# KennyRotella/delta_graph_slam

Hardware: AMD Instinct MI355X
Metric: scan registrations/sec (64k-pt pairs) (higher is better)
Workload: dtype f32 per-point, f64 accumulate; 1 GPU; cfg2 KITTI HDL-64E-shaped pairs (65,536 pts after voxel filter), NDT res 1.0 m DIRECT7, eps 0.01, max 64 iterations; 32 candidate pairs per GPU per step against one target (LoopDetector::matching, cfg4 shard), 32 distinct source scans, fitness score per candidate; inputs resident on the device before timing -- the 35 MB working set of a step fits the 256 MB Infinity Cache, so re-reads between eval; pairs_per_gpu=32, distinct_scans=32, parallelism=candidates sharded one process per GPU, all_gather of result records, collective_world_size=1

## Files before the change

### delta_graph_slam_amd/_lib.py

```python
from __future__ import annotations

import ctypes as C
import os

_HERE = os.path.dirname(os.path.abspath(__file__))
LIB_PATH = os.environ.get("DGS_REG_LIB") or os.path.join(_HERE, "libdgs_reg.so")

DGS_OK = 0
STATUS = {0: "DGS_OK", 1: "DGS_ERR_INVALID_ARGUMENT", 2: "DGS_ERR_HIP", 3: "DGS_ERR_NO_TARGET", 4: "DGS_ERR_NO_SOURCE",
          5: "DGS_ERR_GRID_TOO_LARGE", 6: "DGS_ERR_UNSUPPORTED", 7: "DGS_ERR_CAPACITY"}
DGS_ERR_CAPACITY = 7
METHOD_NDT, METHOD_GICP, METHOD_VGICP, METHOD_ICP, METHOD_PCL_GICP, METHOD_PCL_NDT = 0, 1, 2, 3, 4, 5
VGICP_SEARCH = {"DIRECT1": 0, "DIRECT7": 1, "DIRECT27": 2}
NDT_SEARCH = {"KDTREE": 0, "DIRECT26": 1, "DIRECT7": 2, "DIRECT1": 3}
NDT_ORDER = {"FAST": 0, "UPSTREAM": 1, "UPSTREAM_SEQUENTIAL": 2}
GICP_REG = {"NONE": 0, "MIN_EIG": 1, "NORMALIZED_MIN_EIG": 2, "PLANE": 3, "FROBENIUS": 4}
GICP_COV = {"SYM_EIG": 0, "JACOBI_SVD": 1, "UPSTREAM_ORDER": 2}
K_NDT_DERIVATIVES, K_NDT_SOLVE, K_NDT_VOXEL_BUILD, K_NN_SEARCH, K_GICP_LINEARIZE, K_GICP_COVARIANCE, K_TRANSFORM = range(7)


class DgsError(RuntimeError):
    def __init__(self, status: int, msg: str = ""):
        self.status = status
        super().__init__(f"{STATUS.get(status, status)}: {msg}")
# ... 145 lines not shown
PF_DOWNSAMPLE = {"NONE": 0, "VOXELGRID": 1, "APPROX_VOXELGRID": 2}
PF_OUTLIER = {"NONE": 0, "STATISTICAL": 1, "RADIUS": 2}
PF_NORM_ORDER = {"PAIRS_XY_ZW": 0, "PAIRS_XZ_YW": 1, "SEQUENTIAL": 2}


class Result(C.Structure):
    _fields_ = [("final_transformation", C.c_float * 16), ("converged", C.c_int32), ("iterations", C.c_int32),
                ("evaluations", C.c_int32), ("status", C.c_int32), ("score", C.c_double), ("fitness", C.c_double)]


SYMBOLS = [
    "dgs_params_init", "dgs_create", "dgs_destroy", "dgs_last_error", "dgs_abi_version", "dgs_set_stream",
    "dgs_synchronize", "dgs_set_input_target", "dgs_set_input_source", "dgs_align", "dgs_get_fitness_score",
    "dgs_get_inlier_fraction", "dgs_nearest_search_target", "dgs_nn_fitness_distances", "dgs_align_batch", "dgs_find_loop_candidates", "dgs_calc_fitness_score", "dgs_voxel_grid_filter", "dgs_approx_voxel_grid_filter", "dgs_cloud_create", "dgs_cloud_destroy", "dgs_cloud_size",
    "dgs_set_input_target_cloud", "dgs_set_input_source_cloud", "dgs_align_batch_clouds", "dgs_align_pairs_clouds", "dgs_profile_enable",
    "dgs_profile_get", "dgs_profile_reset", "dgs_get_counts", "dgs_ndt_derivatives", "dgs_ndt_hessian_double", "dgs_ndt_score_gradient", "dgs_deal_probe", "dgs_deal_probe_cost", "dgs_pcl_ndt_neighbours", "dgs_ndt_get_voxels",
    "dgs_ndt_get_trajectory", "dgs_gicp_get_covariances", "dgs_gicp_linearize", "dgs_vgicp_get_voxels",
    "dgs_group_create", "dgs_group_destroy", "dgs_group_last_error", "dgs_group_size", "dgs_group_uses_rccl", "dgs_group_rccl_ranks", "dgs_group_last_gather_used_rccl",
    "dgs_group_member", "dgs_group_set_input_target", "dgs_group_align_batch",
    "dgs_group_cloud_create", "dgs_group_cloud_destroy", "dgs_group_cloud_size", "dgs_group_cloud_copies", "dgs_group_cloud_trim", "dgs_group_set_input_target_cloud",
    "dgs_group_align_batch_clouds",
    "dgs_icp_options_init", "dgs_set_icp_options", "dgs_group_set_icp_options", "dgs_icp_get_trajectory",
    "dgs_pcl_gicp_options_init", "dgs_set_pcl_gicp_options", "dgs_group_set_pcl_gicp_options", "dgs_pcl_gicp_get_trajectory",
    "dgs_pcl_gicp_set_probe", "dgs_pcl_gicp_evaluate", "dgs_pcl_gicp_set_correspondence_randomness",
    "dgs_set_batch_independent", "dgs_get_batch_independent", "dgs_group_set_batch_independent",
    "dgs_prefilter_params_init", "dgs_prefilter", "dgs_prefilter_distance", "dgs_prefilter_radius", "dgs_prefilter_statistical",
    "dgs_prefilter_normal", "dgs_prefilter_get_statistics", "dgs_prefilter_get_normals",
    "dgs_prefilter_scan_params_init", "dgs_prefilter_scan", "dgs_prefilter_deskew",
    "dgs_map_cloud_params_init", "dgs_map_cloud_generate", "dgs_map_cloud_generate_clouds", "dgs_map_cloud_get", "dgs_map_cloud_get_grid",
    "dgs_line_extraction_params_init", "dgs_line_extraction", "dgs_line_extraction_get_rounds",
    "dgs_line_align_params_init", "dgs_line_align_global", "dgs_line_merge", "dgs_line_edges", "dgs_line_align_get_hypotheses",
# ... 63 lines not shown
    lib.dgs_cloud_size.argtypes = [C.c_void_p]
    lib.dgs_cloud_size.restype = C.c_int64
    lib.dgs_set_input_target_cloud.argtypes = [C.c_void_p, C.c_void_p]
    lib.dgs_set_input_source_cloud.argtypes = [C.c_void_p, C.c_void_p]
    lib.dgs_align_batch_clouds.argtypes = [C.c_void_p, C.c_int32, C.c_void_p, C.c_void_p, C.c_int32, C.c_double, P(Result)]
    lib.dgs_align_pairs_clouds.argtypes = [C.c_void_p, C.c_int32, C.c_void_p, C.c_void_p, C.c_void_p, C.c_int32, C.c_double, P(Result)]
    lib.dgs_profile_enable.argtypes = [C.c_void_p, C.c_int32]
    lib.dgs_profile_get.argtypes = [C.c_void_p, C.c_int32, P(C.c_double), P(C.c_int64)]
    lib.dgs_profile_reset.argtypes = [C.c_void_p]
    lib.dgs_get_counts.argtypes = [C.c_void_p, P(C.c_int64)]
    lib.dgs_ndt_derivatives.argtypes = [C.c_void_p, C.c_void_p, C.c_void_p, P(C.c_double), C.c_void_p, C.c_void_p]
    lib.dgs_ndt_hessian_double.argtypes = [C.c_void_p, C.c_void_p, C.c_void_p]
    lib.dgs_ndt_score_gradient.argtypes = [C.c_void_p, C.c_void_p, P(C.c_double), C.c_void_p]
    lib.dgs_deal_probe.argtypes = [C.c_void_p, C.c_void_p, C.c_int32, C.c_int32, C.c_int32, C.c_void_p]
    lib.dgs_deal_probe_cost.argtypes = [C.c_void_p, C.c_void_p, C.c_void_p, C.c_int32, C.c_int32, C.c_int32, C.c_void_p, C.c_void_p]
    lib.dgs_pcl_ndt_neighbours.argtypes = [C.c_void_p, C.c_void_p, C.c_int64, C.c_int32, C.c_void_p, C.c_void_p]
    lib.dgs_ndt_get_voxels.argtypes = [C.c_void_p, P(C.c_int64), C.c_void_p, C.c_void_p, C.c_void_p, C.c_void_p, C.c_void_p]
    lib.dgs_ndt_get_trajectory.argtypes = [C.c_void_p, C.c_int32, C.c_void_p, P(C.c_int32)]
    lib.dgs_gicp_get_covariances.argtypes = [C.c_void_p, C.c_int32, C.c_void_p]
    lib.dgs_gicp_linearize.argtypes = [C.c_void_p, C.c_void_p, C.c_int32, P(C.c_double), C.c_void_p, C.c_void_p]
    lib.dgs_vgicp_get_voxels.argtypes = [C.c_void_p, C.c_int64, C.c_void_p, C.c_void_p, C.c_void_p, C.c_void_p, P(C.c_int64)]
    lib.dgs_group_create.argtypes = [P(Params), C.c_void_p, C.c_int32, P(C.c_void_p)]
    lib.dgs_group_destroy.argtypes = [C.c_void_p]
    lib.dgs_group_destroy.restype = None
    lib.dgs_group_last_error.argtypes = [C.c_void_p]
    lib.dgs_group_last_error.restype = C.c_char_p
    lib.dgs_group_size.argtypes = [C.c_void_p]
    lib.dgs_group_uses_rccl.argtypes = [C.c_void_p]
    lib.dgs_group_rccl_ranks.argtypes = [C.c_void_p]
    lib.dgs_group_last_gather_used_rccl.argtypes = [C.c_void_p]
# ... 108 lines not shown
```

### delta_graph_slam_amd/csrc/dgs_api.hip

```cpp
#include <algorithm>
#include <cfloat>
#include <cmath>
#include <cstddef>
#include <cstdlib>
#include <cstring>
#include <new>
#include <string>
#include <vector>

#include "handle.h"

using namespace dgs;

namespace dgs {

int ensure_pinned(dgs_handle* h, size_t bytes) {
  if (bytes <= h->pinned_bytes) return DGS_OK;
  if (h->pinned) (void)hipHostFree(h->pinned);
  h->pinned = nullptr;
  h->pinned_bytes = 0;
  const size_t want = std::max<size_t>(bytes * 2, 1 << 16);
  hipError_t e = hipHostMalloc(&h->pinned, want, hipHostMallocDefault);
  if (e != hipSuccess) {
    h->err = std::string("hipHostMalloc: ") + hipGetErrorString(e);
// ... 1144 lines not shown
  if (e == hipSuccess) {
    hipLaunchKernelGGL(deal_probe_cost_kernel, dim3(grid), dim3(kBlock), 0, h->stream, d_in.ptr, d_in.ptr + n_pairs, n_pairs, cap_blocks, d_out.ptr);
    e = hipGetLastError();
  }
  if (e == hipSuccess) e = hipMemcpyAsync(out, d_out.ptr, sizeof(int4) * n_out, hipMemcpyDeviceToHost, h->stream);
  if (e == hipSuccess) e = hipStreamSynchronize(h->stream);
  d_in.release();
  d_out.release();
  if (e != hipSuccess) {
    h->err = std::string("dgs_deal_probe_cost: ") + hipGetErrorString(e);
    return DGS_ERR_HIP;
  }
  return DGS_OK;
}

int dgs_find_loop_candidates(dgs_handle* h, const double* accum_distance, const double* xy, int64_t n, int32_t on_device, double new_accum_distance,
                             const double* new_xy, double accum_distance_thresh, double distance_thresh, int32_t* indices, int64_t capacity, int64_t* n_out) {
  if (!h || !n_out || !new_xy || n < 0 || capacity < 0 || (n > 0 && (!accum_distance || !xy)) || (capacity > 0 && !indices) || n > INT32_MAX) return DGS_ERR_INVALID_ARGUMENT;
  h->err.clear();
  if (set_device(h)) return DGS_ERR_HIP;
  *n_out = 0;
  if (n == 0) return DGS_OK;
  dgs::DevBuf<double>& din = h->fc_in;
  dgs::DevBuf<int>& dout = h->fc_out;
  dgs::DevBuf<long long>& dcnt = h->fc_cnt;
  const double* d_acc = accum_distance;
  const double* d_xy = xy;
  int* d_idx = indices;
  const int64_t cap = on_device ? capacity : std::min<int64_t>(capacity, n);
  if (dcnt.reserve(1) != hipSuccess) { h->err = "hipMalloc failed"; return DGS_ERR_HIP; }
// ... 287 lines not shown
```

### delta_graph_slam_amd/csrc/handle.h

```cpp
#pragma once
#include "building_cloud.h"
#include "common.h"
#include "cov_batch_plan.h"
#include "sac.h"

namespace dgs {

struct EventPair {
  hipEvent_t start, stop;
};

struct Profiler {
  bool enabled = false;
  std::vector<EventPair> pool;
  std::vector<int> pending[DGS_K_COUNT];
  std::vector<int> weight;
  size_t next_free = 0;
  double total_ms[DGS_K_COUNT] = {0};
  int64_t launches[DGS_K_COUNT] = {0};
};

struct IcpPair;
struct IcpItem;
struct PgPair;
// ... 519 lines not shown
int stage_host_inputs(dgs_handle* h, DevBuf<float4>& slab, int n, const float* const* inputs, const int64_t* sizes, const float4** d_in);
int ensure_poll_events(dgs_handle* h);
int side_fork(dgs_handle* h);
int side_join(dgs_handle* h);
int side_build_now(dgs_handle* h);

int ndt_build_target(dgs_handle* h);
int voxel_grid_filter(dgs_handle* h, const float4* in, int64_t n, float leaf, float4* out, int64_t out_capacity, int64_t* n_out);
int approx_voxel_grid_filter(dgs_handle* h, const float4* in, int64_t n, float leaf, float4* out, int64_t out_capacity, int64_t* n_out);
int cloud_minmax(dgs_handle* h, const float4* pts, int64_t n, float out6[6]);
int cloud_minmax_device(dgs_handle* h, const float4* pts, int64_t n, float** d_out6, hipStream_t st = nullptr);
int ndt_align_pairs(dgs_handle* h, int n_pairs, const float4* const* d_src_ptrs_host, const int* sizes_host,
                    const float* guesses16, dgs_result* results);
int ndt_trajectory(dgs_handle* h, int pair, double* out, int* len);
int ndt_probe(dgs_handle* h, const double* p6, const float* T16, double* score, double* g6, double* H36, int kind = 1);
inline bool is_pcl_ndt(const dgs_handle* h) { return h->prm.method == DGS_METHOD_PCL_NDT; }
inline bool is_ndt_family(const dgs_handle* h) { return h->prm.method == DGS_METHOD_NDT || h->prm.method == DGS_METHOD_PCL_NDT; }
void pcl_ndt_launch(dgs_handle* h, int n_pairs, int cap_blocks, int total_blocks, int launch, hipStream_t st);
void pcl_ndt_init_tables(dgs_handle* h, int n_pairs, hipStream_t st);
int pcl_ndt_neighbours(dgs_handle* h, const float* queries_xyz16, int64_t m, int on_device, int32_t* counts, int32_t* voxel_ids);
int bvh_build(dgs_handle* h, Bvh& bvh, const float4* pts, int64_t n, hipStream_t st = nullptr, bool kd_order = false);
int nn_fitness(dgs_handle* h, const float4* src, int64_t n, const float* T16, double max_range, double inlier_sq,
               double* sum, int64_t* count, int64_t* inliers);
int nn_fitness_batch(dgs_handle* h, int n_pairs, const float4* const* d_src_ptrs, const int* d_sizes, int max_size, const float* d_T,
                     size_t T_stride_bytes, double max_range, double inlier_sq, double* sums, int64_t* counts, int64_t* inliers);
int nn_fitness_batch_on(dgs_handle* h, const Bvh& index, NnGrid* grid, int n_pairs, const float4* const* d_src_ptrs, const int* d_sizes, int max_size,
                        const float* d_T, size_t T_stride_bytes, double max_range, double inlier_sq, double* sums, int64_t* counts, int64_t* inliers);
int nn_fitness_prepare(dgs_handle* h, int n_pairs, int max_size, bool grid);
void nn_fitness_enqueue(dgs_handle* h, hipStream_t st, const Bvh& index, const int* ids, int count, const float4* const* d_src_ptrs, const int* d_sizes,
                        const float* d_T, size_t T_stride_bytes, double max_range, double inlier_sq, int background_lds_kb);
// ... 108 lines not shown
```

### delta_graph_slam_amd/csrc/ndt_align.hip

```cpp
#include <cfloat>
#include <cmath>
#include <cstdlib>
#include <cstring>

#include "handle.h"
#include "ndt_plan.h"
#include "solve6.h"

namespace dgs {

#include "ndt_fast.h"

#pragma clang fp contract(off)

#include "ndt_exp_tables.h"
#include "ndt_optimiser.h"
#include "ndt_strict.h"
#include "ndt_sequential.h"

__host__ __device__ inline int ndt_queue_slices(int round, int base, int cap) {
  const int f = round < 12 ? 1 : (round < 24 ? 2 : 4);
  return min(base * f, cap);
}
constexpr int kQueueHdrWords = 82;
// ... 739 lines not shown
  if (rc != DGS_OK) return rc;
  const NdtPlan P = plan_align(h);
  launch_derivatives(h, P, L, -1, kind == 2);
  launch_solve(h, P, L);
  char* base = reinterpret_cast<char*>(h->pinned);
  NdtPair* hp = reinterpret_cast<NdtPair*>(base + ((h->pinned_bytes - sizeof(NdtPair) - 64) & ~(size_t)63));
  DGS_HIP_TRY(h, hipMemcpyAsync(hp, h->pairs.ptr, sizeof(NdtPair), hipMemcpyDeviceToHost, st));
  DGS_HIP_TRY(h, hipStreamSynchronize(st));
  DGS_HIP_TRY(h, hipGetLastError());
  *score = hp->s.score;
  for (int k = 0; k < 6; k++) g6[k] = hp->s.grad[k];
  for (int k = 0; k < 36; k++) H36[k] = hp->s.hess[k];
  return DGS_OK;
}

}
```

### delta_graph_slam_amd/csrc/ndt_optimiser.h

```cpp

#ifdef DGS_NDT_PCL_DOUBLE
constexpr bool kNdtDoubleTablesAlways = true;
#else
constexpr bool kNdtDoubleTablesAlways = false;
#endif
template <bool WAVE>
__device__ __forceinline__ void trig6(const double* ang, double* sn, double* cs) {
  if (WAVE) {
    const int lane = threadIdx.x & 63;
    const double a0 = ang[0], a1 = ang[1], a2 = ang[2], a3 = ang[3], a4 = ang[4], a5 = ang[5];
    const double a = (lane == 5) ? a5 : (lane == 4) ? a4 : (lane == 3) ? a3 : (lane == 2) ? a2 : (lane == 1) ? a1 : a0;
    double sv, cv;
    sincos(a, &sv, &cv);
#pragma unroll
    for (int k = 0; k < 6; k++) { sn[k] = readlane_f64(sv, k); cs[k] = readlane_f64(cv, k); }
  } else {
#pragma unroll
    for (int k = 0; k < 6; k++) sincos(ang[k], &sn[k], &cs[k]);
  }
}

template <bool COH>
__device__ __forceinline__ void hdr_put(float* p, float v) {
  if (COH) __hip_atomic_store(p, v, __ATOMIC_RELAXED, __HIP_MEMORY_SCOPE_AGENT);
// ... 457 lines not shown
  if (strict_from_rows) {
    if (pair_blocks[pair] == 0) return;
  }
  __shared__ NdtSolver s_lds;
  NdtSolver& s = s_lds;
  __shared__ double tot[kStrictPad];
  int need_h = 0;
  if (threadIdx.x < kWave) {
    s_lds = st->s;
    need_h = st->need_hessian;
  }
  if (threadIdx.x < kStrictPad) {
    if (strict_from_rows) {
      const int nb = pair_blocks[pair];
      const double* base = partials + (size_t)pair * cap_blocks * kStrictPad + threadIdx.x;
      double v = 0.0;
      for (int b0 = 0; b0 < nb; b0 += 4) {
        double r[4];
#pragma unroll
        for (int k = 0; k < 4; k++) r[k] = base[(size_t)min(b0 + k, nb - 1) * kStrictPad];
#pragma unroll
        for (int k = 0; k < 4; k++)
          if (b0 + k < nb) v += r[k];
      }
      tot[threadIdx.x] = v;
    } else {
      tot[threadIdx.x] = strict_totals[(size_t)pair * kStrictPad + threadIdx.x];
    }
  }
  __syncthreads();
  if (threadIdx.x >= kWave) return;
  const bool writer = threadIdx.x == 0;
  if (need_h != 2) {
    s.score = tot[0];
#pragma unroll
    for (int k = 0; k < 6; k++) s.grad[k] = tot[1 + k];
  }
  if (need_h) {
#pragma unroll
    for (int k = 0; k < 36; k++) s.hess[k] = tot[7 + k];
// ... 13 lines not shown
```

### delta_graph_slam_amd/csrc/ndt_strict.h

```cpp

__device__ __forceinline__ double glibc_exp_dev(double x, const unsigned long long* __restrict__ tab) {
#pragma clang fp contract(off)
  constexpr double N = 128.0;
  constexpr double kInvLn2N = 0x1.71547652b82fep0 * N, kNegLn2hiN = -0x1.62e42fefa0000p-8, kNegLn2loN = -0x1.cf79abc9e3b3ap-47, kShift = 0x1.8p52;
  constexpr double C2 = 0x1.ffffffffffdbdp-2, C3 = 0x1.555555555543cp-3, C4 = 0x1.55555cf172b91p-5, C5 = 0x1.1111167a4d017p-7;
  const unsigned long long xb = (unsigned long long)__double_as_longlong(x);
  const unsigned abstop = (unsigned)(xb >> 52) & 0x7ffu;
  bool special = false;
  if (abstop - 0x3c9u >= 0x408u - 0x3c9u) {
    if (abstop - 0x3c9u >= 0x80000000u) return 1.0 + x;
    if (abstop >= 0x409u) {
      if (xb == 0xfff0000000000000ull) return 0.0;
      if (abstop >= 0x7ffu) return 1.0 + x;
      return (xb >> 63) ? 0.0 : __builtin_inf();
    }
    special = true;
  }
  double kd = __builtin_fma(kInvLn2N, x, kShift);
  const unsigned long long ki = (unsigned long long)__double_as_longlong(kd);
  kd -= kShift;
  const double r = __builtin_fma(kd, kNegLn2loN, __builtin_fma(kd, kNegLn2hiN, x));
  const unsigned idx = 2u * (unsigned)(ki & 127ull);
  const double tail = __longlong_as_double((long long)tab[idx]);
  unsigned long long sbits = tab[idx + 1] + (ki << 45);
// ... 368 lines not shown
  double xj[8], xh[15];
  strict_point_tables_hd(xf, StrictHeader<false>{nullptr, &st}, xj, xh);
  unsigned mask = ROWS ? ((NB >= 32) ? 0xFFFFFFFFu : ((1u << NB) - 1u)) : mask_in;
  while (mask) {
    const int k = __ffs(mask) - 1;
    mask &= mask - 1u;
    bool ok = ((mask_in >> k) & 1u) != 0;
    if (ok) ok = strict_item_hd<ROWS>(xt, xj, xh, vtab + (size_t)strict_pick(vids, k) * 12, gauss_d1, gauss_d2, acc, ROWS ? rows + k : nullptr, row_stride, exptab_d);
    if (ROWS && !ok) {
      for (int en = 0; en < 36; en++) rows[(size_t)en * row_stride + k] = 0.0;
    }
  }
}

constexpr int kStrictRowScratch = 11 * 65;
template <bool COHERENT, bool OWN_SCRATCH = true>
__device__ __forceinline__ void strict_block_row(const double (&acc)[kStrictAccum], const int ncol, double* __restrict__ row_of_slice, double* wave_scratch = nullptr) {
  constexpr int CH = 11, RS = 65, NCH = 4;
  __shared__ double tr[OWN_SCRATCH ? kBlock / kWave : 1][OWN_SCRATCH ? CH * RS : 1];
  __shared__ double sm[kBlock / kWave][kStrictPad];
  const int lane = threadIdx.x & 63, wave = threadIdx.x >> 6;
  double* my = OWN_SCRATCH ? tr[wave] : wave_scratch;
#pragma unroll
  for (int h = 0; h < NCH; h++) {
    if (h * CH >= ncol) break;
#pragma unroll
    for (int k = 0; k < CH; k++) my[k * RS + lane] = (h * CH + k < kStrictAccum) ? acc[h * CH + k < kStrictAccum ? h * CH + k : 0] : 0.0;
    __builtin_amdgcn_wave_barrier();
    __builtin_amdgcn_s_waitcnt(0xc07f);
    if (lane < CH) {
      double v = 0.0;
#pragma unroll 8
      for (int j = 0; j < 64; j++) v += my[lane * RS + j];
// ... 1 lines not shown
    }
    __builtin_amdgcn_wave_barrier();
    __builtin_amdgcn_s_waitcnt(0xc07f);
  }
  __syncthreads();
  if (threadIdx.x < kStrictPad) {
    double v = 0.0;
    if ((int)threadIdx.x < ncol) v = ((sm[0][threadIdx.x] + sm[1][threadIdx.x]) + sm[2][threadIdx.x]) + sm[3][threadIdx.x];
    double* row = row_of_slice + threadIdx.x;
    if (COHERENT) handoff_store_row(row, v);
    else *row = v;
  }
}

constexpr int kStrictSlots = 4;
__device__ __forceinline__ void strict_wave_cols(const double (&acc)[kStrictAccum], const int ncol, double* __restrict__ my, double* __restrict__ cols_of_wave) {
  constexpr int CH = 11, RS = 65, NCH = 4;
  const int lane = threadIdx.x & 63;
#pragma unroll
  for (int h = 0; h < NCH; h++) {
    if (h * CH >= ncol) break;
#pragma unroll
    for (int k = 0; k < CH; k++) my[k * RS + lane] = (h * CH + k < kStrictAccum) ? acc[h * CH + k < kStrictAccum ? h * CH + k : 0] : 0.0;
    __builtin_amdgcn_wave_barrier();
    __builtin_amdgcn_s_waitcnt(0xc07f);
    if (lane < CH) {
      double v = 0.0;
#pragma unroll 8
      for (int j = 0; j < 64; j++) v += my[lane * RS + j];
      cols_of_wave[h * CH + lane] = v;
    }
    __builtin_amdgcn_wave_barrier();
// ... 307 lines not shown
      double xj[8], xh[15];
      strict_table_read_hd<kStrictHdFields, PTS>(td, tdx, (int)(entry >> 25), xt, xj, xh);
      (void)strict_item_hd<false>(xt, xj, xh, row, gauss_d1, gauss_d2, acc, nullptr, 0, exptab_d);
    }
  }
}

constexpr int kStrictSpeculate = 1;
constexpr int kStrictDealByCost = 2;
constexpr int kStrictStampShift = 8;
#ifndef DGS_STRICT_DEAL_BY_COST
#define DGS_STRICT_DEAL_BY_COST 1
#endif

#ifdef DGS_DEAL_STAMPS
constexpr int kStampLaunches = 256, kStampGrid = 2048, kStampWords = 8;
static __device__ unsigned long long* g_deal_stamps;
#define STRICT_DEAL_STAMP_BEGIN                                                                                                        \
  const unsigned long long stamp_t0 = wall_clock64();                                                                                  \
  unsigned long long* const stamp_rec = ((flags >> kStrictStampShift) > 0 && threadIdx.x == 0 && blockIdx.x < kStampGrid && g_deal_stamps) \
      ? g_deal_stamps + ((size_t)((flags >> kStrictStampShift) - 1) * kStampGrid + blockIdx.x) * kStampWords : nullptr;
#define STRICT_DEAL_STAMP_WORK(pair, slice, kind, n_active)                                                                            \
  if (stamp_rec) {                                                                                                                     \
    stamp_rec[0] = stamp_t0;                                                                                                           \
    stamp_rec[1] = wall_clock64();                                                                                                     \
    stamp_rec[3] = (unsigned long long)blockIdx.x | ((unsigned long long)(unsigned)(pair) << 32);                                      \
    stamp_rec[4] = (unsigned long long)(unsigned)((slice) + 1) | ((unsigned long long)(unsigned)(kind) << 32);                         \
    stamp_rec[5] = (unsigned long long)(unsigned)(n_active) | ((unsigned long long)gridDim.x << 32);                                   \
  }
#define STRICT_DEAL_STAMP_CLOSED if (stamp_rec) stamp_rec[2] = wall_clock64();
#else
#define STRICT_DEAL_STAMP_BEGIN
#define STRICT_DEAL_STAMP_WORK(pair, slice, kind, n_active)
#define STRICT_DEAL_STAMP_CLOSED
#endif

template <int SEARCH, bool WITH_HD, bool RING>
struct StrictTile {
  static constexpr int NB = Offsets<SEARCH>::N;
  static constexpr int PTS = (NB <= 7) ? (WITH_HD ? 128 : 64) : 64;
  static constexpr int PTS_HD = 64;
  static constexpr int kRingOffset = kStrictFields * PTS * 4;
  static constexpr int kFloatBytes = kRingOffset + (RING ? kStrictRingBytes : 0);
  static constexpr int kQueue = PTS * NB;
  static constexpr int kHdQueueBytes = PTS_HD * NB * 4;
  static constexpr bool kHdRing = RING && WITH_HD && DGS_STRICT_HD_ITEMS != 0 && kStrictHdFields * 8 * PTS_HD + 5 * 1024 <= kFloatBytes &&
                                  kHdQueueBytes % 16 == 0 && kHdQueueBytes + 1024 + 3 * 4 * PTS_HD <= kQueue * 4;
  static constexpr int kHdFields = kHdRing ? kStrictHdFields : 23;
  static constexpr int kHdBytes = kHdRing ? kStrictHdFields * 8 * PTS_HD + 5 * 1024 : (23 * 8 + 3 * 4) * PTS_HD;
// ... 80 lines not shown
  static_assert(!TL::kHdRing || TL::kTableBytes == TL::kFloatBytes, "the double pass's ring lives in what the float kinds reserve: no more LDS than without it");
  static_assert(SEARCH != 2 || !WITH_HD || FIXED || sizeof(s_tab) + sizeof(s_queue) == 4 * (14336 + 3584), "the timed instantiation: 78,208 B of LDS per workgroup in all");
  __shared__ unsigned long long s_exp2f[32];
  constexpr bool kLdsHeader = DGS_STRICT_LDS_HEADER != 0 && !FIXED;
  __shared__ __attribute__((aligned(16))) StrictHeaderBlock s_hdr;
  {
    unsigned long long e2 = 0ull;
    if (threadIdx.x < 32) e2 = kGlibcExp2fTab[threadIdx.x];
    strict_header_word_t hw = 0u;
    const bool mine = kLdsHeader && !solver && strict_header_load(st, WITH_HD && kind == 2, hw);
    if (threadIdx.x < 32) s_exp2f[threadIdx.x] = e2;
    if (kLdsHeader) strict_header_store(&s_hdr, mine, hw);
  }
  const StrictHeader<kLdsHeader> hdr_wg{(strict_header_lds_t)&s_hdr, &st};
  __syncthreads();
  const unsigned long long* __restrict__ exptab = s_exp2f;
  const unsigned long long* __restrict__ exptab_d = kGlibcExpTab;
  const int lane = threadIdx.x & 63, wave = __builtin_amdgcn_readfirstlane((int)(threadIdx.x >> 6));
  float* tf = reinterpret_cast<float*>(s_tab[wave]);
  float4* ring = reinterpret_cast<float4*>(s_tab[wave] + TL::kRingOffset);
  unsigned* queue = s_queue[wave];
  double* td = reinterpret_cast<double*>(s_tab[wave]);
  float4* ring_hd = reinterpret_cast<float4*>(s_tab[wave] + TL::kHdFields * 8 * TL::PTS_HD);
  float4* ring_hd5 = reinterpret_cast<float4*>(reinterpret_cast<unsigned char*>(queue) + TL::kHdQueueBytes);
  float* tdx = TL::kHdRing ? reinterpret_cast<float*>(reinterpret_cast<unsigned char*>(queue) + TL::kHdQueueBytes + 1024)
                           : reinterpret_cast<float*>(s_tab[wave] + 23 * 8 * TL::PTS_HD);
  const int pts = (WITH_HD && kind == 2) ? TL::PTS_HD : TL::PTS;
  if (solver && wave == 0) {
    __shared__ NdtSolver s_x;
    NdtPair* scratch = reinterpret_cast<NdtPair*>(s_tab[0]);
// ... 5 lines not shown
    __builtin_amdgcn_s_waitcnt(0xc07f);
    __builtin_amdgcn_wave_barrier();
    bool same = queued;
    const int* pub = reinterpret_cast<const int*>(&st);
    const int* mine = reinterpret_cast<const int*>(scratch);
    for (int w = lane; w < 82; w += kWave) same = same && (pub[w] == mine[w]);
    same = __all(same) != 0;
    for (int w = lane; w < kWords; w += kWave)
      __hip_atomic_store(reinterpret_cast<double*>(&pairs[pair].spec_s) + w, reinterpret_cast<const double*>(&s_x)[w], __ATOMIC_RELAXED, __HIP_MEMORY_SCOPE_AGENT);
    if (lane == 0) __hip_atomic_store(&pairs[pair].spec_result, same ? 1 : 2, __ATOMIC_RELAXED, __HIP_MEMORY_SCOPE_AGENT);
    __builtin_amdgcn_wave_barrier();
  }
  const int subs = __builtin_amdgcn_readfirstlane(pts / 64);
  const int stride = __builtin_amdgcn_readfirstlane(n_slices * kBlock);
  static_assert(TL::kTableBytes >= kStrictRowScratch * 8, "the wave's table region doubles as its reduction scratch");
  __shared__ double s_cols[FIXED ? kStrictSlots : 1][FIXED ? kBlock / kWave : 1][FIXED ? kStrictPad : 1];
  static_assert(kStrictSlots * kStrictPad <= kBlock, "one thread per entry of the rows written together");
  int slot = 0, q_first = slice;
#pragma unroll 1
  for (int q = solver ? n_slices : slice; FIXED ? (q < n_slices) : (q == slice && !solver); q += blocks_per_pair) {
#pragma unroll
  for (int k = 0; k < kStrictAccum; k++) acc[k] = 0.0;
#pragma unroll 1
  for (int first = q * kBlock + wave * 64; first < n; first += subs * stride) {
    int qn = 0;
#pragma unroll 1
    for (int sub = 0; sub < subs; sub++) {
      const int i = first + sub * stride + lane;
      const int slot = sub * 64 + lane;
      const StrictHeader<kLdsHeader> hdr = hdr_wg.per_use();
      unsigned mask = 0;
      int vids[NB];
      if (i < n) {
        const float4 x = src[i];
        float xt[3];
        xt[0] = affine_row_rn(T[0], T[1], T[2], T[3], x.x, x.y, x.z);
        xt[1] = affine_row_rn(T[4], T[5], T[6], T[7], x.x, x.y, x.z);
        xt[2] = affine_row_rn(T[8], T[9], T[10], T[11], x.x, x.y, x.z);
        mask = strict_neighbourhood<SEARCH>(xt, g, leaf_pow2, vids);
        if (mask) {
// ... 19 lines not shown
              for (int f = 6; f < 15; f++) tf[(5 + f) * TL::PTS + slot] = xh[f];
            }
          }
        }
      }
#pragma unroll
      for (int k = 0; k < NB; k++) {
        const bool has = (mask >> k) & 1u;
        const unsigned long long b = __ballot(has);
        if (has) queue[qn + __builtin_amdgcn_mbcnt_hi((unsigned)(b >> 32), __builtin_amdgcn_mbcnt_lo((unsigned)b, 0u))] = ((unsigned)slot << 25) | (unsigned)vids[k];
        qn += __popcll(b);
      }
    }
    __builtin_amdgcn_s_waitcnt(0xc07f);
    __builtin_amdgcn_wave_barrier();
    if (!(WITH_HD && kind == 2)) {
      if (kind == 1) strict_items_float<true, TL::PTS, !FIXED>(tf, ring, queue, qn, lane, vs, gauss_d1, gd2, acc, exptab);
      else strict_items_float<false, TL::PTS, !FIXED>(tf, ring, queue, qn, lane, vs, gauss_d1, gd2, acc, exptab);
      qn = 0;
    }
    if (TL::kHdRing && kind == 2) {
      strict_items_hd<TL::PTS_HD>(td, tdx, ring_hd, ring_hd5, queue, qn, lane, vtab, gauss_d1, gauss_d2, acc, exptab_d);
      qn = 0;
    }
#pragma unroll 1
    for (int h = 0; h < qn; h += 64) {
      const int idx = h + lane;
      if (idx < qn) {
        const unsigned entry = queue[idx];
        const int slot = (int)(entry >> 25), vid = (int)(entry & 0x1FFFFFFu);
// ... 3 lines not shown
          strict_table_read_hd<23, TL::PTS_HD>(td, tdx, slot, xt, xj, xh);
          (void)strict_item_hd<false>(xt, xj, xh, vtab + (size_t)vid * 12, gauss_d1, gauss_d2, acc, nullptr, 0, exptab_d);
        } else {
          float xt[3], xj[8], xh[15];
          if (kind == 1) {
            strict_table_read<true, TL::PTS>(tf, slot, xt, xj, xh);
            strict_item<true, true>(xt, xj, xh, vs + vid, gauss_d1, gd2, acc, exptab);
          } else {
            strict_table_read<false, TL::PTS>(tf, slot, xt, xj, xh);
            strict_item<false, true>(xt, xj, xh, vs + vid, gauss_d1, gd2, acc, exptab);
          }
        }
      }
    }
    __builtin_amdgcn_wave_barrier();
  }
  if (FIXED) {
    strict_wave_cols(acc, kind ? kStrictAccum : 7, td, s_cols[slot][wave]);
    slot++;
    if (slot == kStrictSlots || q + blocks_per_pair >= n_slices) {
      strict_rows_flush<FUSED>(reinterpret_cast<const double (*)[kBlock / kWave][kStrictPad]>(&s_cols[0][0][0]), slot, kind ? kStrictAccum : 7,
                               partials + (size_t)pair * cap_blocks * kStrictPad, q_first, blocks_per_pair);
      slot = 0;
      q_first = q + blocks_per_pair;
    }
  } else {
    strict_block_row<FUSED, false>(acc, kind ? kStrictAccum : 7, partials + ((size_t)pair * cap_blocks + slice) * kStrictPad, td);
  }
  }
  if (!FUSED) return;
  __shared__ int s_last;
  if (threadIdx.x < kStrictPad) handoff_drain_stores();
  __syncthreads();
  STRICT_DEAL_STAMP_WORK(pair, slice, kind, n_active)
  const int n_tickets = blocks_per_pair + ((speculate && st.spec_pending) ? 1 : 0);
  if (threadIdx.x == 0) s_last = handoff_take_ticket(&pairs[pair].ticket, n_tickets) ? 1 : 0;
  __syncthreads();
  if (!s_last) return;
#ifdef DGS_CLOSE_STAMPS
  if (threadIdx.x == 0 && pairs[pair].s.nr_iterations == 1) pairs[pair].traj[kTrajCap - 1][5] = (double)wall_clock64();
#endif
  ndt_close_strict<false, WITH_HD>(pairs + pair, partials + (size_t)pair * cap_blocks * kStrictPad, n_slices, consts, done_flags + pair, launch, 1,
                                   solve_min_active > 0 && n_active >= solve_min_active, speculate != 0);
  STRICT_DEAL_STAMP_CLOSED
}

#ifndef DGS_NDT_PCL_DOUBLE
__global__ __launch_bounds__(kWave) void ndt_strict_solve_kernel(NdtPair* __restrict__ pairs, const int n_pairs, const NdtConsts c, int* __restrict__ done_flags, const int launch,
                                                               const int lag) {
  const int pair = blockIdx.x;
  if (pair >= n_pairs) return;
  NdtPair* st = pairs + pair;
// ... 26 lines not shown
```

### include/dgs_reg.h

```cpp
#ifndef DGS_REG_H
#define DGS_REG_H

#include <stdint.h>

#ifdef __cplusplus
extern "C" {
#endif

#define DGS_ABI_VERSION 5

typedef struct dgs_handle dgs_handle;
typedef struct dgs_cloud dgs_cloud;

enum dgs_status {
  DGS_OK = 0,
  DGS_ERR_INVALID_ARGUMENT = 1,
  DGS_ERR_HIP = 2,
  DGS_ERR_NO_TARGET = 3,
  DGS_ERR_NO_SOURCE = 4,
  DGS_ERR_GRID_TOO_LARGE = 5,
  DGS_ERR_UNSUPPORTED = 6,
  DGS_ERR_CAPACITY = 7
};

// ... 186 lines not shown

enum dgs_kernel_id {
  DGS_K_NDT_DERIVATIVES = 0, DGS_K_NDT_SOLVE = 1, DGS_K_NDT_VOXEL_BUILD = 2, DGS_K_NN_SEARCH = 3,
  DGS_K_GICP_LINEARIZE = 4, DGS_K_GICP_COVARIANCE = 5, DGS_K_TRANSFORM = 6, DGS_K_COUNT = 7
};
int dgs_profile_enable(dgs_handle* h, int32_t enable);
int dgs_profile_get(dgs_handle* h, int32_t kernel_id, double* total_ms, int64_t* launches);
int dgs_profile_reset(dgs_handle* h);
int dgs_get_counts(dgs_handle* h, int64_t out[8]);

int dgs_ndt_derivatives(dgs_handle* h, const double* p6, const float* T16, double* score, double* grad6, double* hess36);
int dgs_ndt_hessian_double(dgs_handle* h, const double* p6, double* hess36);
int dgs_ndt_score_gradient(dgs_handle* h, const double* p6, double* score, double* grad6);
int dgs_deal_probe(dgs_handle* h, const int32_t* active, int32_t n_pairs, int32_t cap_blocks, int32_t grid, int32_t* out);
int dgs_deal_probe_cost(dgs_handle* h, const int32_t* active, const int32_t* kinds, int32_t n_pairs, int32_t cap_blocks, int32_t grid, int32_t* out, int32_t* order3);
int dgs_pcl_ndt_neighbours(dgs_handle* h, const float* queries_xyz16, int64_t m, int32_t on_device, int32_t* counts, int32_t* voxel_ids);
int dgs_ndt_get_trajectory(dgs_handle* h, int32_t pair, double* poses6, int32_t* len);
int dgs_icp_get_trajectory(dgs_handle* h, int32_t pair, float* T16s, double* mse, int32_t* n_corr, int32_t capacity, int32_t* len);
int dgs_pcl_gicp_set_probe(dgs_handle* h, const float* T16, const float* guess16);
int dgs_pcl_gicp_evaluate(dgs_handle* h, const double* x6, int32_t* m, double* f, double* g6);
int dgs_pcl_gicp_get_trajectory(dgs_handle* h, int32_t pair, float* T16s, int32_t* n_corr, int32_t* inner, int32_t* passes, double* f,
                                int32_t capacity, int32_t* len);
int dgs_ndt_get_voxels(dgs_handle* h, int64_t* n, int64_t* keys, int32_t* counts, int32_t* valid, double* mean3,
                       double* icov9);

int dgs_nn_fitness_distances(dgs_handle* h, const float* queries_xyz16, int64_t m, int32_t on_device, float* sq_dists);

int dgs_gicp_get_covariances(dgs_handle* h, int32_t which, double* cov9);
int dgs_gicp_linearize(dgs_handle* h, const double* T16_rowmajor, int32_t error_only, double* error, double* hess36, double* b6);
int dgs_vgicp_get_voxels(dgs_handle* h, int64_t capacity, int32_t* coord3, int32_t* counts, double* mean3, double* cov9, int64_t* n_voxels);
// ... 373 lines not shown
```

Before: 7427 registrations/s.

## Reduce strict NDT accumulators in wider 22-column passes and split row summation

```diff
diff --git a/delta_graph_slam_amd/_lib.py b/delta_graph_slam_amd/_lib.py
--- a/delta_graph_slam_amd/_lib.py
+++ b/delta_graph_slam_amd/_lib.py
@@ -183,7 +183,7 @@
     "dgs_synchronize", "dgs_set_input_target", "dgs_set_input_source", "dgs_align", "dgs_get_fitness_score",
     "dgs_get_inlier_fraction", "dgs_nearest_search_target", "dgs_nn_fitness_distances", "dgs_align_batch", "dgs_find_loop_candidates", "dgs_calc_fitness_score", "dgs_voxel_grid_filter", "dgs_approx_voxel_grid_filter", "dgs_cloud_create", "dgs_cloud_destroy", "dgs_cloud_size",
     "dgs_set_input_target_cloud", "dgs_set_input_source_cloud", "dgs_align_batch_clouds", "dgs_align_pairs_clouds", "dgs_profile_enable",
-    "dgs_profile_get", "dgs_profile_reset", "dgs_get_counts", "dgs_ndt_derivatives", "dgs_ndt_hessian_double", "dgs_ndt_score_gradient", "dgs_deal_probe", "dgs_deal_probe_cost", "dgs_pcl_ndt_neighbours", "dgs_ndt_get_voxels",
+    "dgs_profile_get", "dgs_profile_reset", "dgs_get_counts", "dgs_ndt_derivatives", "dgs_ndt_hessian_double", "dgs_ndt_score_gradient", "dgs_deal_probe", "dgs_deal_probe_cost", "dgs_strict_row_probe", "dgs_pcl_ndt_neighbours", "dgs_ndt_get_voxels",
     "dgs_ndt_get_trajectory", "dgs_gicp_get_covariances", "dgs_gicp_linearize", "dgs_vgicp_get_voxels",
     "dgs_group_create", "dgs_group_destroy", "dgs_group_last_error", "dgs_group_size", "dgs_group_uses_rccl", "dgs_group_rccl_ranks", "dgs_group_last_gather_used_rccl",
     "dgs_group_member", "dgs_group_set_input_target", "dgs_group_align_batch",
@@ -277,6 +277,7 @@
     lib.dgs_ndt_score_gradient.argtypes = [C.c_void_p, C.c_void_p, P(C.c_double), C.c_void_p]
     lib.dgs_deal_probe.argtypes = [C.c_void_p, C.c_void_p, C.c_int32, C.c_int32, C.c_int32, C.c_void_p]
     lib.dgs_deal_probe_cost.argtypes = [C.c_void_p, C.c_void_p, C.c_void_p, C.c_int32, C.c_int32, C.c_int32, C.c_void_p, C.c_void_p]
+    lib.dgs_strict_row_probe.argtypes = [C.c_void_p, C.c_void_p, C.c_int32, C.c_void_p]
     lib.dgs_pcl_ndt_neighbours.argtypes = [C.c_void_p, C.c_void_p, C.c_int64, C.c_int32, C.c_void_p, C.c_void_p]
     lib.dgs_ndt_get_voxels.argtypes = [C.c_void_p, P(C.c_int64), C.c_void_p, C.c_void_p, C.c_void_p, C.c_void_p, C.c_void_p]
     lib.dgs_ndt_get_trajectory.argtypes = [C.c_void_p, C.c_int32, C.c_void_p, P(C.c_int32)]
diff --git a/delta_graph_slam_amd/csrc/dgs_api.hip b/delta_graph_slam_amd/csrc/dgs_api.hip
--- a/delta_graph_slam_amd/csrc/dgs_api.hip
+++ b/delta_graph_slam_amd/csrc/dgs_api.hip
@@ -1182,6 +1182,13 @@
   return DGS_OK;
 }
 
+int dgs_strict_row_probe(dgs_handle* h, const double* totals, int32_t ncol, double* rows2) {
+  if (!h || !totals || !rows2 || ncol < 1 || ncol > 43) return DGS_ERR_INVALID_ARGUMENT;
+  h->err.clear();
+  if (set_device(h)) return DGS_ERR_HIP;
+  return strict_row_probe(h, totals, ncol, rows2);
+}
+
 int dgs_find_loop_candidates(dgs_handle* h, const double* accum_distance, const double* xy, int64_t n, int32_t on_device, double new_accum_distance,
                              const double* new_xy, double accum_distance_thresh, double distance_thresh, int32_t* indices, int64_t capacity, int64_t* n_out) {
   if (!h || !n_out || !new_xy || n < 0 || capacity < 0 || (n > 0 && (!accum_distance || !xy)) || (capacity > 0 && !indices) || n > INT32_MAX) return DGS_ERR_INVALID_ARGUMENT;
diff --git a/delta_graph_slam_amd/csrc/handle.h b/delta_graph_slam_amd/csrc/handle.h
--- a/delta_graph_slam_amd/csrc/handle.h
+++ b/delta_graph_slam_amd/csrc/handle.h
@@ -557,6 +557,7 @@
                     const float* guesses16, dgs_result* results);
 int ndt_trajectory(dgs_handle* h, int pair, double* out, int* len);
 int ndt_probe(dgs_handle* h, const double* p6, const float* T16, double* score, double* g6, double* H36, int kind = 1);
+int strict_row_probe(dgs_handle* h, const double* totals, int ncol, double* rows2);
 inline bool is_pcl_ndt(const dgs_handle* h) { return h->prm.method == DGS_METHOD_PCL_NDT; }
 inline bool is_ndt_family(const dgs_handle* h) { return h->prm.method == DGS_METHOD_NDT || h->prm.method == DGS_METHOD_PCL_NDT; }
 void pcl_ndt_launch(dgs_handle* h, int n_pairs, int cap_blocks, int total_blocks, int launch, hipStream_t st);
diff --git a/delta_graph_slam_amd/csrc/ndt_align.hip b/delta_graph_slam_amd/csrc/ndt_align.hip
--- a/delta_graph_slam_amd/csrc/ndt_align.hip
+++ b/delta_graph_slam_amd/csrc/ndt_align.hip
@@ -777,4 +777,33 @@
   return DGS_OK;
 }
 
-}
+__global__ __launch_bounds__(kBlock) void strict_row_probe_kernel(const double* __restrict__ totals, const int ncol, double* __restrict__ rows2) {
+  constexpr int kBytes = StrictTile<DGS_NDT_DIRECT7, true, true>::kTableBytes;
+  __shared__ __attribute__((aligned(16))) unsigned char s_tab[kBlock / kWave][kBytes];
+  double acc[kStrictAccum];
+#pragma unroll
+  for (int k = 0; k < kStrictAccum; k++) acc[k] = totals[(size_t)threadIdx.x * kStrictAccum + k];
+  strict_block_row<false, false, kBytes>(acc, ncol, rows2, reinterpret_cast<double*>(s_tab[threadIdx.x >> 6]));
+  __syncthreads();
+  strict_block_row<false, true>(acc, ncol, rows2 + kStrictPad);
+}
+int strict_row_probe(dgs_handle* h, const double* totals, int ncol, double* rows2) {
+  DevBuf<double> d;
+  const size_t n_in = (size_t)kBlock * kStrictAccum, n_out = 2 * (size_t)kStrictPad;
+  hipError_t e = d.reserve(n_in + n_out);
+  if (e == hipSuccess) e = hipMemcpyAsync(d.ptr, totals, sizeof(double) * n_in, hipMemcpyHostToDevice, h->stream);
+  if (e == hipSuccess) {
+    hipLaunchKernelGGL(strict_row_probe_kernel, dim3(1), dim3(kBlock), 0, h->stream, d.ptr, ncol, d.ptr + n_in);
+    e = hipGetLastError();
+  }
+  if (e == hipSuccess) e = hipMemcpyAsync(rows2, d.ptr + n_in, sizeof(double) * n_out, hipMemcpyDeviceToHost, h->stream);
+  if (e == hipSuccess) e = hipStreamSynchronize(h->stream);
+  d.release();
+  if (e != hipSuccess) {
+    h->err = std::string("dgs_strict_row_probe: ") + hipGetErrorString(e);
+    return DGS_ERR_HIP;
+  }
+  return DGS_OK;
+}
+
+}
diff --git a/delta_graph_slam_amd/csrc/ndt_optimiser.h b/delta_graph_slam_amd/csrc/ndt_optimiser.h
--- a/delta_graph_slam_amd/csrc/ndt_optimiser.h
+++ b/delta_graph_slam_amd/csrc/ndt_optimiser.h
@@ -495,16 +495,24 @@
     if (strict_from_rows) {
       const int nb = pair_blocks[pair];
       const double* base = partials + (size_t)pair * cap_blocks * kStrictPad + threadIdx.x;
-      double v = 0.0;
-      for (int b0 = 0; b0 < nb; b0 += 4) {
-        double r[4];
-#pragma unroll
-        for (int k = 0; k < 4; k++) r[k] = base[(size_t)min(b0 + k, nb - 1) * kStrictPad];
-#pragma unroll
-        for (int k = 0; k < 4; k++)
-          if (b0 + k < nb) v += r[k];
+      constexpr int G = kBlock / kStrictPad;
+      double t = 0.0;
+#pragma unroll 1
+      for (int grp = 0; grp < G; grp++) {
+        double v = 0.0;
+        for (int b0 = grp; b0 < nb; b0 += 4 * G) {
+          double r[4];
+#pragma unroll
+          for (int k = 0; k < 4; k++) {
+            const int b = b0 + k * G;
+            const double x = base[(size_t)min(b, nb - 1) * kStrictPad];
+            r[k] = (b < nb) ? x : 0.0;
+          }
+          v = (((v + r[0]) + r[1]) + r[2]) + r[3];
+        }
+        t += v;
       }
-      tot[threadIdx.x] = v;
+      tot[threadIdx.x] = t;
     } else {
       tot[threadIdx.x] = strict_totals[(size_t)pair * kStrictPad + threadIdx.x];
     }
diff --git a/delta_graph_slam_amd/csrc/ndt_strict.h b/delta_graph_slam_amd/csrc/ndt_strict.h
--- a/delta_graph_slam_amd/csrc/ndt_strict.h
+++ b/delta_graph_slam_amd/csrc/ndt_strict.h
@@ -406,9 +406,15 @@
 }
 
 constexpr int kStrictRowScratch = 11 * 65;
-template <bool COHERENT, bool OWN_SCRATCH = true>
+#ifndef DGS_STRICT_WIDE_ROWS
+#define DGS_STRICT_WIDE_ROWS 1
+#endif
+constexpr int kStrictRowColsWide = 22;
+constexpr int strict_row_cols(const int scratch_bytes) { return (DGS_STRICT_WIDE_ROWS != 0 && scratch_bytes >= kStrictRowColsWide * 65 * 8) ? kStrictRowColsWide : 11; }
+template <bool COHERENT, bool OWN_SCRATCH = true, int SCRATCH_BYTES = 0>
 __device__ __forceinline__ void strict_block_row(const double (&acc)[kStrictAccum], const int ncol, double* __restrict__ row_of_slice, double* wave_scratch = nullptr) {
-  constexpr int CH = 11, RS = 65, NCH = 4;
+  constexpr int CH = OWN_SCRATCH ? 11 : strict_row_cols(SCRATCH_BYTES), RS = 65, NCH = (kStrictAccum + CH - 1) / CH;
+  static_assert(OWN_SCRATCH || CH * RS * 8 <= SCRATCH_BYTES, "a pass fits the scratch the caller hands in");
   __shared__ double tr[OWN_SCRATCH ? kBlock / kWave : 1][OWN_SCRATCH ? CH * RS : 1];
   __shared__ double sm[kBlock / kWave][kStrictPad];
   const int lane = threadIdx.x & 63, wave = threadIdx.x >> 6;
@@ -440,8 +446,10 @@
 }
 
 constexpr int kStrictSlots = 4;
+template <int SCRATCH_BYTES>
 __device__ __forceinline__ void strict_wave_cols(const double (&acc)[kStrictAccum], const int ncol, double* __restrict__ my, double* __restrict__ cols_of_wave) {
-  constexpr int CH = 11, RS = 65, NCH = 4;
+  constexpr int CH = strict_row_cols(SCRATCH_BYTES), RS = 65, NCH = (kStrictAccum + CH - 1) / CH;
+  static_assert(CH * RS * 8 <= SCRATCH_BYTES, "a pass fits the scratch the caller hands in");
   const int lane = threadIdx.x & 63;
 #pragma unroll
   for (int h = 0; h < NCH; h++) {
@@ -779,7 +787,7 @@
 #endif
 
 #ifdef DGS_DEAL_STAMPS
-constexpr int kStampLaunches = 256, kStampGrid = 2048, kStampWords = 8;
+constexpr int kStampLaunches = 256, kStampGrid = 2048, kStampWords = 16;
 static __device__ unsigned long long* g_deal_stamps;
 #define STRICT_DEAL_STAMP_BEGIN                                                                                                        \
   const unsigned long long stamp_t0 = wall_clock64();                                                                                  \
@@ -794,10 +802,29 @@
     stamp_rec[5] = (unsigned long long)(unsigned)(n_active) | ((unsigned long long)gridDim.x << 32);                                   \
   }
 #define STRICT_DEAL_STAMP_CLOSED if (stamp_rec) stamp_rec[2] = wall_clock64();
+#define STRICT_DEAL_STAMP_MARK(word) if (stamp_rec) stamp_rec[word] = wall_clock64();
+#define STRICT_DEAL_STAMP_LAPS_DECL unsigned long long stamp_lap = 0ull, stamp_tiles = 0ull, stamp_items = 0ull;
+#define STRICT_DEAL_STAMP_LAP_BEGIN stamp_lap = wall_clock64();
+#define STRICT_DEAL_STAMP_LAP(total)                                                                                                   \
+  {                                                                                                                                    \
+    const unsigned long long stamp_now = wall_clock64();                                                                               \
+    total += stamp_now - stamp_lap;                                                                                                    \
+    stamp_lap = stamp_now;                                                                                                             \
+  }
+#define STRICT_DEAL_STAMP_LAPS_STORE                                                                                                   \
+  if (stamp_rec) {                                                                                                                     \
+    stamp_rec[7] = stamp_tiles;                                                                                                        \
+    stamp_rec[8] = stamp_items;                                                                                                        \
+  }
 #else
 #define STRICT_DEAL_STAMP_BEGIN
 #define STRICT_DEAL_STAMP_WORK(pair, slice, kind, n_active)
 #define STRICT_DEAL_STAMP_CLOSED
+#define STRICT_DEAL_STAMP_MARK(word)
+#define STRICT_DEAL_STAMP_LAPS_DECL
+#define STRICT_DEAL_STAMP_LAP_BEGIN
+#define STRICT_DEAL_STAMP_LAP(total)
+#define STRICT_DEAL_STAMP_LAPS_STORE
 #endif
 
 template <int SEARCH, bool WITH_HD, bool RING>
@@ -908,6 +935,8 @@
   }
   const StrictHeader<kLdsHeader> hdr_wg{(strict_header_lds_t)&s_hdr, &st};
   __syncthreads();
+  STRICT_DEAL_STAMP_MARK(6)
+  STRICT_DEAL_STAMP_LAPS_DECL
   const unsigned long long* __restrict__ exptab = s_exp2f;
   const unsigned long long* __restrict__ exptab_d = kGlibcExpTab;
   const int lane = threadIdx.x & 63, wave = __builtin_amdgcn_readfirstlane((int)(threadIdx.x >> 6));
@@ -943,6 +972,10 @@
   const int subs = __builtin_amdgcn_readfirstlane(pts / 64);
   const int stride = __builtin_amdgcn_readfirstlane(n_slices * kBlock);
   static_assert(TL::kTableBytes >= kStrictRowScratch * 8, "the wave's table region doubles as its reduction scratch");
+  static_assert(DGS_STRICT_WIDE_ROWS == 0 || TL::kTableBytes < kStrictRowColsWide * 65 * 8 || strict_row_cols(TL::kTableBytes) == kStrictRowColsWide,
+                "a table region of 22 x 65 doubles or more is reduced in passes of 22 columns");
+  static_assert(DGS_STRICT_WIDE_ROWS == 0 || SEARCH != 2 || !WITH_HD || FIXED || strict_row_cols(TL::kTableBytes) == kStrictRowColsWide, "the timed instantiation: two passes");
+
   __shared__ double s_cols[FIXED ? kStrictSlots : 1][FIXED ? kBlock / kWave : 1][FIXED ? kStrictPad : 1];
   static_assert(kStrictSlots * kStrictPad <= kBlock, "one thread per entry of the rows written together");
   int slot = 0, q_first = slice;
@@ -953,6 +986,7 @@
 #pragma unroll 1
   for (int first = q * kBlock + wave * 64; first < n; first += subs * stride) {
     int qn = 0;
+    STRICT_DEAL_STAMP_LAP_BEGIN
 #pragma unroll 1
     for (int sub = 0; sub < subs; sub++) {
       const int i = first + sub * stride + lane;
@@ -1002,6 +1036,7 @@
     }
     __builtin_amdgcn_s_waitcnt(0xc07f);
     __builtin_amdgcn_wave_barrier();
+    STRICT_DEAL_STAMP_LAP(stamp_tiles)
     if (!(WITH_HD && kind == 2)) {
       if (kind == 1) strict_items_float<true, TL::PTS, !FIXED>(tf, ring, queue, qn, lane, vs, gauss_d1, gd2, acc, exptab);
       else strict_items_float<false, TL::PTS, !FIXED>(tf, ring, queue, qn, lane, vs, gauss_d1, gd2, acc, exptab);
@@ -1035,9 +1070,11 @@
       }
     }
     __builtin_amdgcn_wave_barrier();
-  }
+    STRICT_DEAL_STAMP_LAP(stamp_items)
+  }
+  STRICT_DEAL_STAMP_MARK(9)
   if (FIXED) {
-    strict_wave_cols(acc, kind ? kStrictAccum : 7, td, s_cols[slot][wave]);
+    strict_wave_cols<TL::kTableBytes>(acc, kind ? kStrictAccum : 7, td, s_cols[slot][wave]);
     slot++;
     if (slot == kStrictSlots || q + blocks_per_pair >= n_slices) {
       strict_rows_flush<FUSED>(reinterpret_cast<const double (*)[kBlock / kWave][kStrictPad]>(&s_cols[0][0][0]), slot, kind ? kStrictAccum : 7,
@@ -1046,10 +1083,12 @@
       q_first = q + blocks_per_pair;
     }
   } else {
-    strict_block_row<FUSED, false>(acc, kind ? kStrictAccum : 7, partials + ((size_t)pair * cap_blocks + slice) * kStrictPad, td);
+    strict_block_row<FUSED, false, TL::kTableBytes>(acc, kind ? kStrictAccum : 7, partials + ((size_t)pair * cap_blocks + slice) * kStrictPad, td);
   }
   }
   if (!FUSED) return;
+  STRICT_DEAL_STAMP_MARK(10)
+  STRICT_DEAL_STAMP_LAPS_STORE
   __shared__ int s_last;
   if (threadIdx.x < kStrictPad) handoff_drain_stores();
   __syncthreads();
@@ -1057,6 +1096,7 @@
   const int n_tickets = blocks_per_pair + ((speculate && st.spec_pending) ? 1 : 0);
   if (threadIdx.x == 0) s_last = handoff_take_ticket(&pairs[pair].ticket, n_tickets) ? 1 : 0;
   __syncthreads();
+  STRICT_DEAL_STAMP_MARK(11)
   if (!s_last) return;
 #ifdef DGS_CLOSE_STAMPS
   if (threadIdx.x == 0 && pairs[pair].s.nr_iterations == 1) pairs[pair].traj[kTrajCap - 1][5] = (double)wall_clock64();
diff --git a/include/dgs_reg.h b/include/dgs_reg.h
--- a/include/dgs_reg.h
+++ b/include/dgs_reg.h
@@ -224,6 +224,7 @@
 int dgs_ndt_score_gradient(dgs_handle* h, const double* p6, double* score, double* grad6);
 int dgs_deal_probe(dgs_handle* h, const int32_t* active, int32_t n_pairs, int32_t cap_blocks, int32_t grid, int32_t* out);
 int dgs_deal_probe_cost(dgs_handle* h, const int32_t* active, const int32_t* kinds, int32_t n_pairs, int32_t cap_blocks, int32_t grid, int32_t* out, int32_t* order3);
+int dgs_strict_row_probe(dgs_handle* h, const double* totals, int32_t ncol, double* rows2);
 int dgs_pcl_ndt_neighbours(dgs_handle* h, const float* queries_xyz16, int64_t m, int32_t on_device, int32_t* counts, int32_t* voxel_ids);
 int dgs_ndt_get_trajectory(dgs_handle* h, int32_t pair, double* poses6, int32_t* len);
 int dgs_icp_get_trajectory(dgs_handle* h, int32_t pair, float* T16s, double* mse, int32_t* n_corr, int32_t capacity, int32_t* len);
```

Result: faster. 7553 registrations/s (median of 6 runs) (+1.7%).
